# auggiemarignier/pxmcmc

Measured on AMD Instinct MI355X. Metric: MYULA samples/sec at L=256 synthesis, higher is better.
Workload: dtype f64

## Files before the change

include/pxmcmc_amd.h:

```cpp
#ifndef PXMCMC_AMD_H
#define PXMCMC_AMD_H

#include <stddef.h>
#include <stdint.h>

#ifdef __cplusplus
extern "C" {
#endif

typedef struct pxm_sht_plan_s* pxm_sht_plan_t;
typedef struct pxm_wav_plan_s* pxm_wav_plan_t;
typedef struct pxm_dwav_plan_s* pxm_dwav_plan_t;
typedef struct pxm_hwav_plan_s* pxm_hwav_plan_t;
typedef void* pxm_stream_t;

int pxm_version(void);
#ifdef PXM_NOISE_F64
#error "the -DPXM_NOISE_F64 build switch was removed: pass the flag PXM_NOISE_F64 per call (one library serves both precisions)"
#endif
#define PXM_NOISE_F64 16
int pxm_noise_bits(void);
int64_t pxm_host_check_address_ranges(int L, double B, int J_min, int spin, int max_chains, int what);
const char* pxm_last_error(void);
int pxm_device_count(void);

int pxm_capture_begin(void);
int pxm_capture_end(void);
int pxm_deferred_pending(void);
int pxm_tables_trim(void);

int pxm_j_max(int L, double B);
int pxm_wav_bandlimits(int L, double B, int J_min, int* bl_out, int cap);
int64_t pxm_wav_ncoefs(int L, double B, int J_min, int64_t* nscal_out);
int pxm_tiling_axisym(int L, double B, int J_min, double* kappa0, double* kappa);
int pxm_mw_ring_weights(int L, double* q);
int pxm_host_sht_tables(int L, int spin, int m, double* Binv, double* Afwd);
int pxm_host_rec_table(int L, int spin, int m, double* Brec);
// ... 160 lines not shown
```

pxmcmc_amd/_lib.py:

```python
import ctypes as C
import os

import torch

_HERE = os.path.dirname(os.path.abspath(__file__))
LIB_PATH = os.environ.get("PXM_LIB_PATH") or os.path.join(_HERE, "lib", "libpxmcmc_amd.so")

c_i64, c_u64, c_int, c_dbl, c_vp = C.c_int64, C.c_uint64, C.c_int, C.c_double, C.c_void_p

SIGNATURES = {
    "pxm_version": (c_int, []),
    "pxm_noise_bits": (c_int, []),
    "pxm_host_check_address_ranges": (c_i64, [c_int, c_dbl, c_int, c_int, c_int, c_int]),
    "pxm_last_error": (C.c_char_p, []),
    "pxm_device_count": (c_int, []),
    "pxm_capture_begin": (c_int, []),
    "pxm_capture_end": (c_int, []),
    "pxm_deferred_pending": (c_int, []),
    "pxm_tables_trim": (c_int, []),
    "pxm_wav_set_iter_counter": (c_int, [c_vp, c_vp]),
    "pxm_wav_release_iter_counter": (c_int, [c_vp, c_vp]),
    "pxm_wav_iter_counter_add": (c_int, [c_vp, c_u64, c_vp]),
    "pxm_wav_exact_dft_scales": (c_int, [c_vp]),
    "pxm_wav_status": (c_int, [c_vp, c_int, c_vp]),
    "pxm_sht_status": (c_int, [c_vp, c_int, c_vp]),
    "pxm_wav_profile_enable": (c_int, [c_vp, c_int]),
    "pxm_wav_profile_read": (c_int, [c_vp, c_vp, c_vp, c_vp, c_vp]),
    "pxm_wav_profile_read_launches": (c_int, [c_vp, c_vp, c_vp, c_vp, c_i64, c_vp]),
# ... 154 lines not shown
```

pxmcmc_amd/csrc/plans.hip:

```cpp
#include "../../include/pxmcmc_amd.h"
#include "elem.h"
#include "sht_core.h"
#include "sht_rec.h"

#include <algorithm>
#include <cmath>
#include <cstdlib>
#include <cstring>
#include <map>
#include <string>
#include <memory>
#include <mutex>

namespace pxm {

struct TaskList {
  GemmTask* d = nullptr;
  int n = 0;
  bool paired = false;
  int nslab = 2;
  std::vector<int> bls;
  std::vector<int> los;
  double mfma_units = 0;
  bool gram = false;
// ... 82 lines not shown
      if (!any) break;
    }
    v.swap(ordered);
  }
  out->n = (int)v.size();
  out->paired = paired;
  out->nslab = pk ? 4 : (paired ? 2 : 1);
  for (const GemmTask& t : v) {
    PXM_REQUIRE(t.n_rt >= 0 && t.n_rt <= 8 && t.row0 >= 0 && t.row0 % 16 == 0 && t.k_beg >= 0 && t.k_beg % 16 == 0 &&
                    (t.n_rt == 0 || (t.k_end > t.k_beg && (t.k_end - t.k_beg) % 16 == 0)),
                "upload_tasks: malformed GEMM task");
    out->mfma_units += (double)t.n_rt * ((t.k_end - t.k_beg) / 4) * (pk ? 1 : t.nslab);
    for (int sl = 0; sl < 4; ++sl)
      if (t.x2_off[sl]) out->flags |= 1;
    if (t.ks_off[0] || t.ks_off[1]) out->flags |= 2;
  }
  if (v.empty()) return 0;
  if (int rc = check_gemm_task_ranges(v, out->nslab, out->flags, ncol, ws_base, name)) return rc;
  if (int rc = dev_alloc(&out->d, v.size() * sizeof(GemmTask), "GEMM task list")) return rc;
  return dev_upload(out->d, v.data(), v.size() * sizeof(GemmTask));
}

static double tasklist_bytes(const TaskList& tl, int cg) {
  double bytes = 0;
  for (size_t i = 0; i < tl.bls.size(); ++i) {
    const double Ld = tl.bls[i];
    if (tl.gram) bytes += tl.gram_table_bytes + 3 * 16.0 * cg * Ld * Ld + 16.0 * Ld * Ld;
    else bytes += gemm_alg_bytes(tl.bls[i], tl.paired, cg, tl.los[i]);
    if (!tl.gram && tl.pk && tl.tab_shared[i]) bytes -= gemm_table_bytes(tl.bls[i], tl.paired, tl.los[i]);
  }
// ... 238 lines not shown
  double B = 0;
  int nsc = 0;
  std::vector<int> bl;
  std::vector<int64_t> coef_off;
  int64_t ncoefs = 0;
  std::vector<ShtTables*> T;
  ShtTables* TL = nullptr;
  std::vector<DftPlan> dft;
  DftPlan dftL;
  double* ws = nullptr;
  std::vector<int64_t> offG;
  int64_t offGL = 0, offHL = 0, offS = 0;
  int64_t offGD = 0, offHD = 0;
  int64_t offHDc = 0;
  TaskList gram, adj_invadj_D;
  bool have_data_rings = false;
  int64_t offHA = 0, offHB = 0;
  double* d_kc_syn = nullptr;
  double* d_kc_ana = nullptr;
  TaskList syn_fwd, syn_inv, adj_invadj, adj_fwdadj;
  TaskList ana_fwd, ana_inv, anadj_invadj, anadj_fwdadj;
  int64_t table_bytes[2] = {0, 0};
  static constexpr int NSIDE = 3;
  static constexpr int nside = 2;
  hipStream_t side[NSIDE] = {nullptr, nullptr, nullptr};
  hipEvent_t ev_fork = nullptr, ev_join[NSIDE] = {nullptr, nullptr, nullptr};
  bool plain_group = true;
  std::vector<int> lane_of;
  DftGroupList dft_group;
  int pk = 0;
// ... 257 lines not shown

int pxm_wav_plan_create_spin(int L, double B, int J_min, int spin, int max_chains, unsigned flags, pxm_wav_plan_t* plan) {
  (void)flags;
  return wav_plan_create_impl("pxm_wav_plan_create_spin", L, B, J_min, spin, max_chains, plan);
}

int pxm_wav_plan_destroy(pxm_wav_plan_t p) {
  if (!p) return 0;
  dft_group_destroy(&p->dft_group);
  for (auto& d : p->dft) free_dft_plan(&d);
  free_dft_plan(&p->dftL);
  deferred_free(p->ws);
  deferred_free(p->d_kc_syn);
  deferred_free(p->d_kc_ana);
  deferred_free(p->d_wlk);
  deferred_free(p->d_status);
  TaskList* tls[] = {&p->syn_fwd, &p->syn_inv, &p->adj_invadj, &p->adj_fwdadj, &p->gram, &p->adj_invadj_D,
                     &p->ana_fwd, &p->ana_inv, &p->anadj_invadj, &p->anadj_fwdadj, &p->wl_inv, &p->wl_invadj};
  for (TaskList* t : tls) free_tasks(t);
  profiler_release(&p->prof);
  for (ShtTables* T : p->held) release_tables(T);
  rec_tables_destroy(p->rec2);
  deferred_free(p->d_twin);
  deferred_free(p->d_g2n);
  deferred_free(p->d_hn);
  deferred_free(p->d_gn);
  dft_group_destroy(&p->dft_group_n);
  free_tasks(&p->wl_syn_fwd);
  free_tasks(&p->wl_adj_fwdadj);
  delete p;
// ... 353 lines not shown
  if ((rc = launch_ring2px(p->dftL, p->ws + p->offGL, p->ncol, po, C, st))) return rc;
  return pxm_wav_image_init(p, preds_out, data, invcov, invcov_complex, C, stream);
}

}
namespace pxm {
__global__ void k_pack_data_term(const double2* __restrict__ HD, double2* __restrict__ HDc, int64_t rows, int Cp) {
  for (int64_t i = blockIdx.x * (int64_t)blockDim.x + threadIdx.x; i < rows; i += (int64_t)gridDim.x * blockDim.x) HDc[i] = HD[i * Cp];
}
}
extern "C" {

static int wav_make_gram_lists(pxm_wav_plan_t p) {
  int rc;
  if (!p->gram.d) {
    if ((rc = get_tables(p->L, p->spin, 1u << TAB_GRAM, &p->TL))) return rc;
    wav_hold(p, p->TL);
    std::vector<GemmTask> v;
    GemmFuse fz;
    fz.x2_base = p->offHB;
    fz.hd_base = p->offHDc;
    fz.hd_stride = 2;
    append_gemm_tasks(*p->TL, TAB_GRAM, p->ncol, p->offHA, p->L, p->Rp, p->offHL, p->L, p->Rp, nullptr, p->offS, p->ws, v, 0, fz);
    if ((rc = upload_tasks(v, p->TL->paired, &p->gram, {p->L}, p->ncol, p->ws, "Gram step"))) return rc;
    p->gram.gram = true;
    p->gram.gram_table_bytes = (double)p->TL->bytes[TAB_GRAM];
    v.clear();
    append_gemm_tasks(*p->TL, TAB_INV_ADJ, p->ncol, p->offGD, p->L, p->Rp, p->offHD, p->L, p->Rp, nullptr, p->offS, p->ws, v);
    if ((rc = upload_tasks(v, p->TL->paired, &p->adj_invadj_D, {p->L}, p->ncol, p->ws, "inverse-adjoint of the data rings"))) return rc;
  }
  return 0;
}

int pxm_wav_ring_set_data(pxm_wav_plan_t p, const void* data, pxm_stream_t stream) {
  PXM_REQUIRE(p && data, "pxm_wav_ring_set_data: null argument");
  hipStream_t st = (hipStream_t)stream;
  int rc;
  if ((rc = wav_make_gram_lists(p))) return rc;
  PxIn in;
  in.f = (const double*)data;
  in.chain_stride = (int64_t)p->L * (2 * p->L - 1);
// ... 232 lines not shown

int pxm_wav_analysis_adjoint(pxm_wav_plan_t p, const void* X, void* f, int C, pxm_stream_t stream) {
  int rc = wav_check(p, X, f, C, "pxm_wav_analysis_adjoint");
  if (rc) return rc;
  hipStream_t st = (hipStream_t)stream;
  if ((rc = wav_blocks_to_rings(p, X, C, st))) return rc;
  if ((rc = run_tasks(p->anadj_invadj, p->ws, p->ws, p->ncol, C, st, GemmAffine(), &p->prof))) return rc;
  if ((rc = run_tasks(p->anadj_fwdadj, p->ws, p->ws, p->ncol, C, st, GemmAffine(), &p->prof))) return rc;
  PxOut out;
  out.f = (double*)f;
  out.chain_stride = (int64_t)p->L * (2 * p->L - 1);
  return launch_ring2px(p->dftL, p->ws + p->offGL, p->ncol, out, C, st);
}

int64_t pxm_wav_table_bytes(pxm_wav_plan_t p, int op) {
  if (!p || op < 0 || op > 1) return -1;
  return p->table_bytes[op];
}

int64_t pxm_host_check_address_ranges(int L, double B, int J_min, int spin, int max_chains, int what) {
  static std::mutex mu;
  std::lock_guard<std::mutex> lock(mu);
  PXM_REQUIRE(!capture_in_progress(), "pxm_host_check_address_ranges: not during a stream capture");
  set_dry_run(true);
  ranges_checked_reset();
  int rc = 0;
  if (what & 1) {
    pxm_sht_plan_t sp = nullptr;
    rc = pxm_sht_plan_create(L, spin, max_chains, 0, &sp);
    if (sp) pxm_sht_plan_destroy(sp);
  }
  if (!rc && (what & 2)) {
    pxm_wav_plan_t wp = nullptr;
    const int wspin = (what & 8) ? spin : 0;
    rc = pxm_wav_plan_create_spin(L, B, J_min, wspin, max_chains, 0, &wp);
    if (!rc) rc = wav_make_gram_lists(wp);
    if (!rc && (what & 4) && L >= 3 && wspin == 0) rc = pxm_wav_wl_attach(wp, nullptr, nullptr, (int64_t)L * (2 * L - 1));
    if (wp) pxm_wav_plan_destroy(wp);
  }
  tables_trim();
  set_dry_run(false);
  return rc ? -1 : ranges_checked();
}

}
```

pxmcmc_amd/csrc/sht_core.h:

```cpp
#pragma once
#include "common.h"

namespace pxm {

enum TableKind { TAB_INV = 0, TAB_FWD = 1, TAB_INV_ADJ = 2, TAB_FWD_ADJ = 3, TAB_GRAM = 4, TAB_KINDS = 5 };
inline bool kind_el_to_ring(int kind) { return kind == TAB_INV || kind == TAB_FWD_ADJ; }
inline bool kind_rows_are_el(int kind) { return kind == TAB_FWD || kind == TAB_INV_ADJ || kind == TAB_GRAM; }
inline bool kind_k_is_el(int kind) { return kind == TAB_INV || kind == TAB_FWD_ADJ || kind == TAB_GRAM; }

struct GemmTask {
  int64_t tab_off;
  int64_t rt_stride;
  int64_t x_off[4];
  int64_t y_off[4];
  int64_t x2_off[4];
  int64_t hd_off[4];
  int64_t ks_off[2];
  int64_t rs_off[2];
  int row_lo[2], row_hi[2];
  int k_beg, k_end;
  int row0;
  int n_rt;
  int nslab;
  double sign1;
  int m_unit;
  int hd_stride;
  int x_ncol, y_ncol;
};

struct GemmAffine {
  double ns = 0, wr = 0, wi = 0;
  int on = 0;
  int ncol_live = 1 << 30;
  uint64_t* bump = nullptr;
};

struct Profiler {
  struct Pool {
    std::vector<std::pair<hipEvent_t, hipEvent_t>> ev;
    size_t used = 0;
    double bytes = 0, flops = 0;
    std::vector<double> launch_bytes;
// ... 19 lines not shown
                  int32_t* per_launch_wgs = nullptr);
void profiler_release(Profiler* pr);

struct GemmFuse {
  int64_t x2_base = -1;
  const double* rscale = nullptr;
  int row_lo = 0, row_hi = 1 << 30;
  int64_t hd_base = -1;
  int hd_stride = 0;
};

struct ShtTables {
  int L = 0, spin = 0, Rp = 0;
  bool paired = false;
  int n_m = 0;
  double* d_tab[TAB_KINDS] = {nullptr, nullptr, nullptr, nullptr, nullptr};
  size_t bytes[TAB_KINDS] = {0, 0, 0, 0, 0};
  std::vector<int64_t> m_off[TAB_KINDS];
  std::vector<int> k_beg[TAB_KINDS];
  int refs = 0;
  int m_of(int i) const { return paired ? i : i - (L - 1); }
};

int get_tables(int L, int spin, unsigned kinds_mask, ShtTables** out);
void retain_tables(ShtTables* T);
void release_tables(ShtTables* T);
int64_t tables_trim();

void append_gemm_tasks(const ShtTables& T, int kind, int ncol, int64_t x_base, int x_L, int x_Rp,
                       int64_t y_base, int y_L, int y_Rp, const double* kscale, int64_t scratch_off,
                       const double* ws_base, std::vector<GemmTask>& tasks, int el_lo = 0,
                       const GemmFuse& fuse = GemmFuse());
struct GemmSide {
  int64_t x_base, y_base;
  int x_L, x_Rp, y_L, y_Rp;
  const double* kscale;
  int el_lo;
  GemmFuse fuse;
  int x_ncol = 0, y_ncol = 0;
};

void append_gemm_tasks_packed(const ShtTables& T, int kind, int ncol, const GemmSide& side_a, const GemmSide* side_b,
                              int64_t scratch_off, const double* ws_base, std::vector<GemmTask>& tasks);
int launch_gemm_packed(const GemmTask* d_tasks, int n_tasks, int pk, int flags, const double* X, double* Y, int ncol, int col0,
                       double alg_bytes, double flops, hipStream_t stream, Profiler* prof = nullptr);

int launch_gemm(const GemmTask* d_tasks, int n_tasks, int nslab, int flags, const double* X, double* Y, int ncol,
                int col0, int ct, double alg_bytes, double flops, hipStream_t stream,
                const GemmAffine& aff = GemmAffine(), Profiler* prof = nullptr);

inline double gemm_table_bytes(int L, bool paired, int el_lo = 0) {
  double tab_entries = 0;
  for (int m = paired ? 0 : -(L - 1); m < L; ++m) {
    const int am = m < 0 ? -m : m;
    const int n = L - (am > el_lo ? am : el_lo);
// ... 111 lines not shown
```

pxmcmc_amd/csrc/sht_gemm.hip:

```cpp
#include "../../include/pxmcmc_amd.h"
#include "sht_core.h"

#include <type_traits>

#include <hip/hip_ext.h>

#include <cstdlib>
#include <map>
#include <mutex>

namespace pxm {

typedef double d4 __attribute__((ext_vector_type(4)));

constexpr int KC = 16;
#define PXM_GEMM_MFMA(ACC, A, B) ACC = __builtin_amdgcn_mfma_f64_16x16x4f64(A, B, ACC, 0, 0, 0);
#ifdef PXM_GEMM_TRACE
__device__ unsigned long long* g_gemm_trace = nullptr;
extern "C" int pxm_debug_set_gemm_trace(unsigned long long* buf) {
  return hipMemcpyToSymbol(HIP_SYMBOL(g_gemm_trace), &buf, sizeof(buf)) == hipSuccess ? 0 : -1;
}
#endif
__device__ __forceinline__ double stage_add(double a, double b, bool on) { return a + (on ? b : 0.0); }
__device__ __forceinline__ double2 stage_add(double2 a, double2 b, bool on) { return double2{a.x + (on ? b.x : 0.0), a.y + (on ? b.y : 0.0)}; }
// ... 8 lines not shown
template <int CT, int NSLAB, int NW, int RT, int NSET, bool TWO, bool SK, int PK = 0>
__device__ __forceinline__ void sht_gemm_body(const GemmTask* __restrict__ tasks, const int bid,
                                              const double* __restrict__ X, double* __restrict__ Y, int ncol, int col0,
                                              const GemmAffine& aff, double (*xs)[KC][GemmGeom<CT, NSLAB>::PITCH]) {
  constexpr int NCT = CT * NSLAB;
  constexpr bool HOIST = TWO;
  constexpr int COLS = GemmGeom<CT, NSLAB>::COLS;
  constexpr int PITCH = GemmGeom<CT, NSLAB>::PITCH;
  constexpr int NT = 64 * NW;
  constexpr int VW = (KC * COLS / 2 >= NT) ? 2 : 1;
  constexpr int NV = KC * COLS / VW;
  constexpr int IT = (NV + NT - 1) / NT;
  const GemmTask t = tasks[bid];
  const int tid = threadIdx.x, lane = tid & 63;
  if (t.n_rt == 0) return;
  const int xn = PK ? t.x_ncol : ncol, yn = PK ? t.y_ncol : ncol;
#ifdef PXM_GEMM_TRACE
  const unsigned long long trace_t0 = wall_clock64();
  unsigned long long trace_t1 = 0, trace_t2 = 0;
  long long trace_c[5] = {0, 0, 0, 0, 0};
#define PXM_GEMM_CSTAMP(K) if (ch == 8) trace_c[K] = clock64();
#else
#define PXM_GEMM_CSTAMP(K)
#endif
  const int wave = __builtin_amdgcn_readfirstlane(tid >> 6);
  const int kq = lane >> 4, cl = lane & 15;
  const int n_my = min(RT, max(0, t.n_rt - RT * wave));
  const int nch = (t.k_end - t.k_beg) / KC;

  const double* sp[IT];
  const double* sp2[IT];
// ... 12 lines not shown
    sp[i] = X + xo + col0 + cin + (int64_t)(t.k_beg + kr) * xn;
    sp2[i] = sp[i];
    skp[i] = sp[i];
    if (TWO) {
      const int64_t x2o = tasks[bid].x2_off[slab];
      if (x2o) sp2[i] = sp[i] + (x2o - xo);
    }
    if (SK) {
      const int64_t ks = tasks[bid].ks_off[slab >> 1];
      if (ks) skp[i] = X + ks + t.k_beg + kr;
    }
    so[i] = kr * PITCH + col;
  }
  const bool two = TWO && t.x2_off[0] != 0;
  const bool has_sk = SK && t.ks_off[0] != 0;
  typedef typename std::conditional<VW == 2, double2, double>::type stage_t;
  stage_t st[NSET - 1][IT], st2[NSET - 1][IT];
  double ssc[NSET - 1][IT];
#define PXM_STAGE_LOAD(SET, CH)                                                                     \
  {                                                                                                 \
    const int cs = min((CH), nch - 1);                                                              \
    _Pragma("unroll") for (int i = 0; i < IT; ++i) {                                                \
      st[SET][i] = *reinterpret_cast<const stage_t*>(sp[i] + (int64_t)cs * KC * xn);                \
      if (TWO) st2[SET][i] = *reinterpret_cast<const stage_t*>(sp2[i] + (int64_t)cs * KC * xn);   \
      if (SK) ssc[SET][i] = skp[i][cs * KC];                                                        \
    }                                                                                               \
  }
#define PXM_STAGE_STORE(SET, BUF)                                                                   \
  _Pragma("unroll") for (int i = 0; i < IT; ++i) {                                                  \
    stage_t v = st[SET][i];                                                                         \
// ... 73 lines not shown
  }
        PXM_MFMA_CHUNK(NCT)
#undef PXM_MFMA_CHUNK
      }
      PXM_GEMM_CSTAMP(3)
    }
  }
#undef PXM_STAGE_LOAD
#undef PXM_STAGE_STORE
#undef PXM_TAB_LOAD
#ifdef PXM_GEMM_TRACE
  trace_t2 = wall_clock64();
#endif

  constexpr int NGRP = PK ? 2 : 1;
  double hdv[RT][NSLAB][4], rsv[RT][NGRP][4];
#pragma unroll
  for (int r = 0; r < RT; ++r) {
    const int rowb = t.row0 + 16 * (r < n_my ? RT * wave + r : 0) + kq;
#pragma unroll
    for (int sl = 0; sl < NSLAB; ++sl)
#pragma unroll
      for (int q = 0; q < 4; ++q)
        hdv[r][sl][q] = (aff.on && t.hd_off[sl]) ? (X + t.hd_off[sl])[(int64_t)(rowb + 4 * q) * t.hd_stride + (cl & 1)] : 0.0;
#pragma unroll
    for (int g = 0; g < NGRP; ++g)
#pragma unroll
      for (int q = 0; q < 4; ++q) rsv[r][g][q] = t.rs_off[g] ? (X + t.rs_off[g])[rowb + 4 * q] : 1.0;
  }
  if constexpr (PK != 0) {
    const int slab = cl / PK, grp = slab >> 1;
    const bool live = slab < t.nslab;
    const double sgn = (slab & 1) ? t.sign1 : 1.0;
    const int64_t yo = tasks[bid].y_off[live ? slab : 0];
    const int row_lo = grp ? t.row_lo[1] : t.row_lo[0], row_hi = grp ? t.row_hi[1] : t.row_hi[0];
#pragma unroll
    for (int r = 0; r < RT; ++r) {
      if (r >= n_my) continue;
      const int rowb = t.row0 + 16 * (RT * wave + r) + kq;
      double* yb = Y + yo + col0 + (cl % PK) + (int64_t)rowb * yn;
#pragma unroll
      for (int q = 0; q < 4; ++q) {
        const int row = rowb + 4 * q;
        const double rs = grp ? rsv[r][NGRP - 1][q] : rsv[r][0][q];
        if (live && row >= row_lo && row < row_hi) yb[(int64_t)(4 * q) * yn] = sgn * rs * acc[r][0][q];
      }
    }
  } else {
#pragma unroll
  for (int r = 0; r < RT; ++r) {
    if (r >= n_my) continue;
#pragma unroll
    for (int c = 0; c < NCT; ++c) {
      const int slab = c / CT, cin = 16 * (c % CT), grp = slab >> 1;
      const double sgn = (slab & 1) ? t.sign1 : 1.0;
      const int rowb = t.row0 + 16 * (RT * wave + r) + kq;
      double* yb = Y + t.y_off[slab] + col0 + cin + cl + (int64_t)rowb * ncol;
#pragma unroll
      for (int q = 0; q < 4; ++q) {
        const int row = rowb + 4 * q;
        double v = acc[r][c][q];
        if (aff.on) {
          const double u = aff.ns * v - hdv[r][slab][q];
          int lo = __double2loint(u), hi = __double2hiint(u);
          lo = __builtin_amdgcn_mov_dpp(lo, 0xB1, 0xF, 0xF, true);
          hi = __builtin_amdgcn_mov_dpp(hi, 0xB1, 0xF, 0xF, true);
          const double pu = __hiloint2double(hi, lo);
          v = (cl & 1) ? (aff.wr * u + aff.wi * pu) : (aff.wr * u - aff.wi * pu);
          if (col0 + cin + cl >= aff.ncol_live) v = 0.0;
        }
        if (row >= t.row_lo[grp] && row < t.row_hi[grp]) yb[(int64_t)(4 * q) * ncol] = sgn * rsv[r][grp][q] * v;
      }
    }
  }
  }
#ifdef PXM_GEMM_TRACE
  __syncthreads();
  if (tid == 0 && g_gemm_trace) {
    unsigned hw, xcc;
    asm volatile("s_getreg_b32 %0, hwreg(HW_REG_HW_ID)" : "=s"(hw));
    asm volatile("s_getreg_b32 %0, hwreg(HW_REG_XCC_ID)" : "=s"(xcc));
    const unsigned long long slot = atomicAdd(g_gemm_trace, 1ull);
    unsigned long long* r = g_gemm_trace + 8 + 8 * slot;
    r[0] = blockIdx.x; r[1] = gridDim.x; r[2] = trace_t0; r[3] = wall_clock64();
    r[4] = ((unsigned long long)(xcc & 0xf) << 32) | hw; r[5] = (unsigned long long)nch | ((unsigned long long)t.n_rt << 16) | ((unsigned long long)aff.on << 32);
    r[6] = trace_t1; r[7] = trace_t2;
// ... 85 lines not shown
    return -1;
  };
  auto ok = [&](int64_t lo, int64_t hi) {
    ++n;
    return lo <= hi && dev_range_ok(ws_base + lo, ws_base + hi + 1, &why);
  };
  const bool TWO = flags & 1, SK = flags & 2;
  for (size_t ti = 0; ti < v.size(); ++ti) {
    const GemmTask& t = v[ti];
    if (t.n_rt == 0) continue;
    const int nch = (t.k_end - t.k_beg) / KC;
    if (!ok(t.tab_off, t.tab_off + (int64_t)(t.n_rt - 1) * t.rt_stride + (int64_t)(2 * (nch - 1) + 1) * 128 + 127))
      return bad(ti, "ring-table stream", 0);
    for (int col0 = 0; col0 < ncol; col0 += 32) {
      const int CT = (ncol - col0 >= 32) ? 2 : 1;
      for (int slab = 0; slab < nslab; ++slab) {
        const int xn = t.x_ncol ? t.x_ncol : ncol, yn = t.y_ncol ? t.y_ncol : ncol;
        const int wx = std::min(16 * CT, xn), wy = std::min(16 * CT, yn);
        const int64_t lo = col0 + (int64_t)t.k_beg * xn, hi = col0 + wx - 1 + (int64_t)(t.k_end - 1) * xn;
        if (!ok(t.x_off[slab] + lo, t.x_off[slab] + hi)) return bad(ti, "operand staging", col0);
        if (TWO && t.x2_off[slab] && !ok(t.x2_off[slab] + lo, t.x2_off[slab] + hi)) return bad(ti, "second operand staging", col0);
        if (SK && t.ks_off[slab >> 1] && !ok(t.ks_off[slab >> 1] + t.k_beg, t.ks_off[slab >> 1] + t.k_end - 1))
          return bad(ti, "operand scale vector", col0);
        const int64_t r_lo = t.row0, r_hi = t.row0 + 16 * t.n_rt - 1;
        if (t.hd_off[slab] && !ok(t.hd_off[slab] + r_lo * t.hd_stride, t.hd_off[slab] + r_hi * t.hd_stride + 1))
          return bad(ti, "affine data term", col0);
        if (t.rs_off[slab >> 1] && !ok(t.rs_off[slab >> 1] + r_lo, t.rs_off[slab >> 1] + r_hi))
          return bad(ti, "per-row output scale", col0);
        const int64_t s_lo = std::max<int64_t>(r_lo, t.row_lo[slab >> 1]), s_hi = std::min<int64_t>(r_hi, (int64_t)t.row_hi[slab >> 1] - 1);
        if (s_lo <= s_hi && !ok(t.y_off[slab] + col0 + s_lo * yn, t.y_off[slab] + col0 + wy - 1 + s_hi * yn))
// ... 115 lines not shown
    const int n_rt_total = (Rp - row_beg) / 16;
    for (int rt = 0; rt < n_rt_total; rt += rpt) {
      GemmTask g;
      g.m_unit = T.paired ? m : m + T.L - 1;
      g.tab_off = (T.d_tab[kind] + T.m_off[kind][i] + tab_skip + (int64_t)rt * rt_stride) - ws_base;
      g.rt_stride = rt_stride;
      for (int s = 0; s < 2; ++s) fill_side(g, s, T, kind, m, ncol, side, scratch_off, ws_base);
      g.nslab = T.paired ? 2 : 1;
      g.k_beg = k_beg;
      g.k_end = k_end;
      g.row0 = row_beg + 16 * rt;
      g.n_rt = std::min(rpt, n_rt_total - rt);
      g.sign1 = (kind == TAB_GRAM) ? 1.0 : ((m & 1) ? -1.0 : 1.0);
      g.x_ncol = side.x_ncol ? side.x_ncol : ncol;
      g.y_ncol = side.y_ncol ? side.y_ncol : ncol;
      tasks.push_back(g);
    }
  }
}

void append_gemm_tasks_packed(const ShtTables& T, int kind, int ncol, const GemmSide& side_a, const GemmSide* side_b,
                              int64_t scratch_off, const double* ws_base, std::vector<GemmTask>& tasks) {
  GemmSide sa = side_a;
  if (side_b) sa.el_lo = std::min(side_a.el_lo, side_b->el_lo);
  const size_t first = tasks.size();
  append_tasks_impl(T, kind, ncol, sa, scratch_off, ws_base, tasks);
  for (size_t i = first; i < tasks.size(); ++i) {
    GemmTask& g = tasks[i];
    const int m = T.paired ? g.m_unit : g.m_unit - (T.L - 1);
    fill_side(g, 0, T, kind, m, ncol, side_a, scratch_off, ws_base);
    fill_side(g, 1, T, kind, m, ncol, side_b ? *side_b : side_a, scratch_off, ws_base);
    g.nslab = side_b ? 4 : 2;
// ... 22 lines not shown
  const double* Q = Qd + (int64_t)par * Rp * Rp;
  double acc = 0;
  for (int tp = 0; tp < L; ++tp) acc += B[(int64_t)tp * Rp + el] * Q[(int64_t)tp * Rp + t];
  Ad[(int64_t)i * Rp * Rp + (int64_t)el * Rp + t] = scale * acc;
}

__global__ void k_build_gram(const double* __restrict__ Bd, double* __restrict__ Gd, int Rp, int L) {
  const int i = blockIdx.z;
  const int r = blockIdx.x * 16 + threadIdx.x, c = blockIdx.y * 16 + threadIdx.y;
  const double* B = Bd + (int64_t)i * Rp * Rp;
  double acc = 0;
  for (int t = 0; t < L; ++t) acc += B[(int64_t)t * Rp + r] * B[(int64_t)t * Rp + c];
  Gd[(int64_t)i * Rp * Rp + (int64_t)r * Rp + c] = acc;
}

__global__ void k_tile_table(const double* __restrict__ D, double* __restrict__ out, int Rp, int row_beg,
                             int k_beg, int transposed) {
  const int nk2 = (Rp - k_beg) / 8;
  const int rt = blockIdx.y;
  const int kk2 = blockIdx.x;
  const int lane = threadIdx.x >> 1, h = threadIdx.x & 1;
  const int row = row_beg + 16 * rt + (lane & 15);
  const int k = k_beg + 8 * kk2 + 4 * h + (lane >> 4);
  const double v = transposed ? D[(int64_t)k * Rp + row] : D[(int64_t)row * Rp + k];
  out[((int64_t)rt * nk2 + kk2) * 128 + threadIdx.x] = v;
}

static std::mutex g_tab_mutex;
static std::map<std::pair<int, int>, ShtTables*> g_tab_cache;

static int build_kind(ShtTables& T, int kind, const double* d_B, const double* d_A, const double* d_G) {
  const int Rp = T.Rp;
  const bool rows_el = kind_rows_are_el(kind), k_el = kind_k_is_el(kind);
  T.m_off[kind].resize(T.n_m);
  T.k_beg[kind].resize(T.n_m);
  int64_t total = 0;
  for (int i = 0; i < T.n_m; ++i) {
    const int elmin = std::max(std::abs(T.m_of(i)), std::abs(T.spin));
    const int kb = round_down(elmin, 16);
    T.k_beg[kind][i] = kb;
    T.m_off[kind][i] = total;
    total += (int64_t)((rows_el ? Rp - kb : Rp) / 16) * ((k_el ? Rp - kb : Rp) / 8) * 128;
  }
  T.bytes[kind] = (size_t)total * sizeof(double);
  if (int rc = dev_alloc(&T.d_tab[kind], T.bytes[kind], "ring table")) return rc;
  if (dry_run()) return 0;
  for (int i = 0; i < T.n_m; ++i) {
    const int kb = T.k_beg[kind][i];
    const double* src;
    int transposed;
    if (kind == TAB_INV) { src = d_B; transposed = 0; }
// ... 35 lines not shown
  unsigned missing = 0;
  for (int k = 0; k < TAB_KINDS; ++k)
    if ((kinds_mask >> k & 1u) && !T->d_tab[k]) missing |= 1u << k;
  if (missing && dry_run()) {
    for (int k = 0; k < TAB_KINDS; ++k)
      if (missing >> k & 1u) {
        int rc = build_kind(*T, k, nullptr, nullptr, nullptr);
        if (rc) return rc;
      }
  } else if (missing) {
    const int Rp = T->Rp;
    const size_t dense = (size_t)T->n_m * Rp * Rp;
    std::vector<double> hB(dense, 0.0);
    const int m0 = T->paired ? 0 : -(L - 1);
    for (int i = 0; i < T->n_m; ++i) wigner_ring_table(L, spin, m0 + i, hB.data() + (size_t)i * Rp * Rp, Rp);
    double *d_B = nullptr, *d_A = nullptr, *d_Q = nullptr, *d_G = nullptr;
    PXM_HIP(hipMalloc(&d_B, dense * sizeof(double)));
    PXM_HIP(hipMemcpy(d_B, hB.data(), dense * sizeof(double), hipMemcpyHostToDevice));
    hB.clear();
    hB.shrink_to_fit();
    if (missing & ((1u << TAB_FWD) | (1u << TAB_FWD_ADJ))) {
      std::vector<double> hQ((size_t)2 * Rp * Rp, 0.0);
      quadrature_gram(L, +1, hQ.data(), Rp);
      quadrature_gram(L, -1, hQ.data() + (size_t)Rp * Rp, Rp);
      PXM_HIP(hipMalloc(&d_Q, hQ.size() * sizeof(double)));
      PXM_HIP(hipMemcpy(d_Q, hQ.data(), hQ.size() * sizeof(double), hipMemcpyHostToDevice));
      PXM_HIP(hipMalloc(&d_A, dense * sizeof(double)));
      dim3 grid(Rp / 16, Rp / 16, T->n_m), block(16, 16);
      hipLaunchKernelGGL(k_build_fwd, grid, block, 0, 0, d_B, d_Q, d_A, Rp, L, 2.0 * M_PI / (2 * L - 1), m0, spin);
      PXM_HIP(hipGetLastError());
    }
    if (missing & (1u << TAB_GRAM)) {
      PXM_HIP(hipMalloc(&d_G, dense * sizeof(double)));
      dim3 grid(Rp / 16, Rp / 16, T->n_m), block(16, 16);
      hipLaunchKernelGGL(k_build_gram, grid, block, 0, 0, d_B, d_G, Rp, L);
      PXM_HIP(hipGetLastError());
    }
    for (int k = 0; k < TAB_KINDS; ++k)
      if (missing >> k & 1u) {
        int rc = build_kind(*T, k, d_B, d_A, d_G);
        if (rc) return rc;
      }
    PXM_HIP(hipDeviceSynchronize());
    PXM_HIP(hipFree(d_B));
    if (d_A) PXM_HIP(hipFree(d_A));
    if (d_Q) PXM_HIP(hipFree(d_Q));
    if (d_G) PXM_HIP(hipFree(d_G));
  }
  *out = T;
  return 0;
}

void retain_tables(ShtTables* T) {
  std::lock_guard<std::mutex> lock(g_tab_mutex);
  if (T) ++T->refs;
}
void release_tables(ShtTables* T) {
  std::lock_guard<std::mutex> lock(g_tab_mutex);
  if (T && T->refs > 0) --T->refs;
}
int64_t tables_trim() {
  std::lock_guard<std::mutex> lock(g_tab_mutex);
// ... 20 lines not shown
```

Baseline: 115,300.

## Split spin-0 Gram table by degree parity with a rank-one pole correction

For spin 0 and L divisible by 32, the Gram step uses a new table kind that keeps only the even-even and odd-odd degree blocks of each per-m Gram matrix. The GEMM tasks stride over the interleaved rows (row_step 2), and for m=0 a rank-one pole correction is computed in shared memory and added in the epilogue. Large m near Rp stay dense. The goal is to roughly halve Gram table bytes and FLOPs in the MYULA step, at the cost of extra kernel complexity, a shared-memory reduction for m=0, and an environment variable switch.

```diff
diff --git a/include/pxmcmc_amd.h b/include/pxmcmc_amd.h
--- a/include/pxmcmc_amd.h
+++ b/include/pxmcmc_amd.h
@@ -21,6 +21,7 @@
 #define PXM_NOISE_F64 16
 int pxm_noise_bits(void);
 int64_t pxm_host_check_address_ranges(int L, double B, int J_min, int spin, int max_chains, int what);
+int64_t pxm_host_gram_table_bytes(int L, int spin, int* parity);
 const char* pxm_last_error(void);
 int pxm_device_count(void);
 
diff --git a/pxmcmc_amd/_lib.py b/pxmcmc_amd/_lib.py
--- a/pxmcmc_amd/_lib.py
+++ b/pxmcmc_amd/_lib.py
@@ -12,6 +12,7 @@
     "pxm_version": (c_int, []),
     "pxm_noise_bits": (c_int, []),
     "pxm_host_check_address_ranges": (c_i64, [c_int, c_dbl, c_int, c_int, c_int, c_int]),
+    "pxm_host_gram_table_bytes": (c_i64, [c_int, c_int, C.POINTER(c_int)]),
     "pxm_last_error": (C.c_char_p, []),
     "pxm_device_count": (c_int, []),
     "pxm_capture_begin": (c_int, []),
diff --git a/pxmcmc_amd/csrc/plans.hip b/pxmcmc_amd/csrc/plans.hip
--- a/pxmcmc_amd/csrc/plans.hip
+++ b/pxmcmc_amd/csrc/plans.hip
@@ -120,6 +120,8 @@
     for (int sl = 0; sl < 4; ++sl)
       if (t.x2_off[sl]) out->flags |= 1;
     if (t.ks_off[0] || t.ks_off[1]) out->flags |= 2;
+    PXM_REQUIRE(pk || t.n_rt == 0 || ((t.row_step == 1 || t.row_step == 2) && t.x_ncol == ncol * t.row_step && t.y_ncol == ncol * t.row_step),
+                "upload_tasks: a task's row stride differs from row_step * ncol");
   }
   if (v.empty()) return 0;
   if (int rc = check_gemm_task_ranges(v, out->nslab, out->flags, ncol, ws_base, name)) return rc;
@@ -388,6 +390,8 @@
   int64_t offGD = 0, offHD = 0;
   int64_t offHDc = 0;
   TaskList gram, adj_invadj_D;
+  bool gram_parity = false;
+  double* d_pole = nullptr;
   bool have_data_rings = false;
   int64_t offHA = 0, offHB = 0;
   double* d_kc_syn = nullptr;
@@ -675,6 +679,7 @@
   deferred_free(p->d_kc_syn);
   deferred_free(p->d_kc_ana);
   deferred_free(p->d_wlk);
+  deferred_free(p->d_pole);
   deferred_free(p->d_status);
   TaskList* tls[] = {&p->syn_fwd, &p->syn_inv, &p->adj_invadj, &p->adj_fwdadj, &p->gram, &p->adj_invadj_D,
                      &p->ana_fwd, &p->ana_inv, &p->anadj_invadj, &p->anadj_fwdadj, &p->wl_inv, &p->wl_invadj};
@@ -1058,17 +1063,30 @@
 static int wav_make_gram_lists(pxm_wav_plan_t p) {
   int rc;
   if (!p->gram.d) {
-    if ((rc = get_tables(p->L, p->spin, 1u << TAB_GRAM, &p->TL))) return rc;
+    const bool par = gram_parity_wanted(p->L, p->spin);
+    const int kind = par ? TAB_GRAM_PAR : TAB_GRAM;
+    p->gram_parity = par;
+    if ((rc = get_tables(p->L, p->spin, 1u << kind, &p->TL))) return rc;
     wav_hold(p, p->TL);
     std::vector<GemmTask> v;
     GemmFuse fz;
     fz.x2_base = p->offHB;
     fz.hd_base = p->offHDc;
     fz.hd_stride = 2;
-    append_gemm_tasks(*p->TL, TAB_GRAM, p->ncol, p->offHA, p->L, p->Rp, p->offHL, p->L, p->Rp, nullptr, p->offS, p->ws, v, 0, fz);
+    if (par) {
+      const int Rh = p->Rp / 2;
+      std::vector<double> u((size_t)p->Rp, 0.0);
+      for (int l = 0; l < p->L; ++l) u[(size_t)(l & 1) * Rh + l / 2] = ((l & 1) ? -1.0 : 1.0) * std::sqrt((2.0 * l + 1.0) / (8.0 * M_PI));
+      if ((rc = dev_alloc(&p->d_pole, u.size() * sizeof(double), "Gram pole vector [2][Rp / 2]"))) return rc;
+      if ((rc = dev_upload(p->d_pole, u.data(), u.size() * sizeof(double)))) return rc;
+      const GemmSide sd{p->offHA, p->offHL, p->L, p->Rp, p->L, p->Rp, nullptr, 0, fz};
+      append_gram_parity_tasks(*p->TL, p->ncol, sd, p->offS, p->d_pole, p->ws, v);
+    } else {
+      append_gemm_tasks(*p->TL, TAB_GRAM, p->ncol, p->offHA, p->L, p->Rp, p->offHL, p->L, p->Rp, nullptr, p->offS, p->ws, v, 0, fz);
+    }
     if ((rc = upload_tasks(v, p->TL->paired, &p->gram, {p->L}, p->ncol, p->ws, "Gram step"))) return rc;
     p->gram.gram = true;
-    p->gram.gram_table_bytes = (double)p->TL->bytes[TAB_GRAM];
+    p->gram.gram_table_bytes = (double)p->TL->bytes[kind];
     v.clear();
     append_gemm_tasks(*p->TL, TAB_INV_ADJ, p->ncol, p->offGD, p->L, p->Rp, p->offHD, p->L, p->Rp, nullptr, p->offS, p->ws, v);
     if ((rc = upload_tasks(v, p->TL->paired, &p->adj_invadj_D, {p->L}, p->ncol, p->ws, "inverse-adjoint of the data rings"))) return rc;
@@ -1331,7 +1349,9 @@
 }
 
 int64_t pxm_wav_table_bytes(pxm_wav_plan_t p, int op) {
-  if (!p || op < 0 || op > 1) return -1;
+  if (!p || op < 0 || op > 3) return -1;
+  if (op == 2) return (int64_t)p->gram.gram_table_bytes;
+  if (op == 3) return p->gram.d ? (p->gram_parity ? 1 : 0) : -1;
   return p->table_bytes[op];
 }
 
@@ -1360,4 +1380,21 @@
   return rc ? -1 : ranges_checked();
 }
 
-}
+int64_t pxm_host_gram_table_bytes(int L, int spin, int* parity) {
+  static std::mutex mu;
+  std::lock_guard<std::mutex> lock(mu);
+  PXM_REQUIRE(L >= 1 && (std::abs(spin) < L || L == 1), "pxm_host_gram_table_bytes: bad (L, spin)");
+  PXM_REQUIRE(!capture_in_progress(), "pxm_host_gram_table_bytes: not during a stream capture");
+  const bool par = gram_parity_wanted(L, spin);
+  const int kind = par ? TAB_GRAM_PAR : TAB_GRAM;
+  set_dry_run(true);
+  ShtTables* T = nullptr;
+  const int rc = get_tables(L, spin, 1u << kind, &T);
+  const int64_t bytes = rc ? -1 : (int64_t)T->bytes[kind];
+  tables_trim();
+  set_dry_run(false);
+  if (parity) *parity = par ? 1 : 0;
+  return bytes;
+}
+
+}
diff --git a/pxmcmc_amd/csrc/sht_core.h b/pxmcmc_amd/csrc/sht_core.h
--- a/pxmcmc_amd/csrc/sht_core.h
+++ b/pxmcmc_amd/csrc/sht_core.h
@@ -3,10 +3,10 @@
 
 namespace pxm {
 
-enum TableKind { TAB_INV = 0, TAB_FWD = 1, TAB_INV_ADJ = 2, TAB_FWD_ADJ = 3, TAB_GRAM = 4, TAB_KINDS = 5 };
+enum TableKind { TAB_INV = 0, TAB_FWD = 1, TAB_INV_ADJ = 2, TAB_FWD_ADJ = 3, TAB_GRAM = 4, TAB_GRAM_PAR = 5, TAB_KINDS = 6 };
 inline bool kind_el_to_ring(int kind) { return kind == TAB_INV || kind == TAB_FWD_ADJ; }
-inline bool kind_rows_are_el(int kind) { return kind == TAB_FWD || kind == TAB_INV_ADJ || kind == TAB_GRAM; }
-inline bool kind_k_is_el(int kind) { return kind == TAB_INV || kind == TAB_FWD_ADJ || kind == TAB_GRAM; }
+inline bool kind_rows_are_el(int kind) { return kind == TAB_FWD || kind == TAB_INV_ADJ || kind == TAB_GRAM || kind == TAB_GRAM_PAR; }
+inline bool kind_k_is_el(int kind) { return kind == TAB_INV || kind == TAB_FWD_ADJ || kind == TAB_GRAM || kind == TAB_GRAM_PAR; }
 
 struct GemmTask {
   int64_t tab_off;
@@ -26,6 +26,10 @@
   int m_unit;
   int hd_stride;
   int x_ncol, y_ncol;
+  int row_step;
+  int64_t pole_u_off;
+  int64_t pole_uo_off;
+  int64_t pole_dx;
 };
 
 struct GemmAffine {
@@ -75,8 +79,8 @@
   int L = 0, spin = 0, Rp = 0;
   bool paired = false;
   int n_m = 0;
-  double* d_tab[TAB_KINDS] = {nullptr, nullptr, nullptr, nullptr, nullptr};
-  size_t bytes[TAB_KINDS] = {0, 0, 0, 0, 0};
+  double* d_tab[TAB_KINDS] = {};
+  size_t bytes[TAB_KINDS] = {};
   std::vector<int64_t> m_off[TAB_KINDS];
   std::vector<int> k_beg[TAB_KINDS];
   int refs = 0;
@@ -100,6 +104,11 @@
   GemmFuse fuse;
   int x_ncol = 0, y_ncol = 0;
 };
+
+void append_gram_parity_tasks(const ShtTables& T, int ncol, const GemmSide& side, int64_t scratch_off, const double* pole_u,
+                              const double* ws_base, std::vector<GemmTask>& tasks);
+bool gram_parity_wanted(int L, int spin);
+inline bool gram_par_dense_m(int Rp, int m) { return m > 0 && m >= Rp - 32; }
 
 void append_gemm_tasks_packed(const ShtTables& T, int kind, int ncol, const GemmSide& side_a, const GemmSide* side_b,
                               int64_t scratch_off, const double* ws_base, std::vector<GemmTask>& tasks);
diff --git a/pxmcmc_amd/csrc/sht_gemm.hip b/pxmcmc_amd/csrc/sht_gemm.hip
--- a/pxmcmc_amd/csrc/sht_gemm.hip
+++ b/pxmcmc_amd/csrc/sht_gemm.hip
@@ -6,6 +6,7 @@
 #include <hip/hip_ext.h>
 
 #include <cstdlib>
+#include <cstring>
 #include <map>
 #include <mutex>
 
@@ -46,7 +47,7 @@
   const GemmTask t = tasks[bid];
   const int tid = threadIdx.x, lane = tid & 63;
   if (t.n_rt == 0) return;
-  const int xn = PK ? t.x_ncol : ncol, yn = PK ? t.y_ncol : ncol;
+  const int xn = PK ? t.x_ncol : ncol * t.row_step, yn = PK ? t.y_ncol : ncol * t.row_step;
 #ifdef PXM_GEMM_TRACE
   const unsigned long long trace_t0 = wall_clock64();
   unsigned long long trace_t1 = 0, trace_t2 = 0;
@@ -89,6 +90,27 @@
   }
   const bool two = TWO && t.x2_off[0] != 0;
   const bool has_sk = SK && t.ks_off[0] != 0;
+
+  constexpr bool POLE = TWO && PK == 0;
+  constexpr int PCW = 16 * CT;
+  __shared__ double pole_red[POLE ? NT : 1], pole_s[POLE ? PCW : 1];
+  const bool pole = POLE && t.pole_u_off != 0;
+  if (pole) {
+    const int pc = tid % PCW, pg = tid / PCW;
+    const double* xq = X + t.x_off[0] + t.pole_dx + col0 + pc;
+    const double* xq2 = two ? X + t.x2_off[0] + t.pole_dx + col0 + pc : xq;
+    const double* uo = X + t.pole_uo_off;
+    double part = 0.0;
+    for (int k = t.k_beg + pg; k < t.k_end; k += NT / PCW) part += uo[k] * (xq[(int64_t)k * xn] + (two ? xq2[(int64_t)k * xn] : 0.0));
+    pole_red[tid] = part;
+    __syncthreads();
+    if (tid < PCW) {
+      double sum = 0.0;
+      for (int g = 0; g < NT / PCW; ++g) sum += pole_red[g * PCW + tid];
+      pole_s[tid] = sum;
+    }
+    __syncthreads();
+  }
   typedef typename std::conditional<VW == 2, double2, double>::type stage_t;
   stage_t st[NSET - 1][IT], st2[NSET - 1][IT];
   double ssc[NSET - 1][IT];
@@ -192,7 +214,7 @@
 #endif
 
   constexpr int NGRP = PK ? 2 : 1;
-  double hdv[RT][NSLAB][4], rsv[RT][NGRP][4];
+  double hdv[RT][NSLAB][4], rsv[RT][NGRP][4], puv[RT][4];
 #pragma unroll
   for (int r = 0; r < RT; ++r) {
     const int rowb = t.row0 + 16 * (r < n_my ? RT * wave + r : 0) + kq;
@@ -205,6 +227,8 @@
     for (int g = 0; g < NGRP; ++g)
 #pragma unroll
       for (int q = 0; q < 4; ++q) rsv[r][g][q] = t.rs_off[g] ? (X + t.rs_off[g])[rowb + 4 * q] : 1.0;
+#pragma unroll
+    for (int q = 0; q < 4; ++q) puv[r][q] = pole ? (X + t.pole_u_off)[rowb + 4 * q] : 0.0;
   }
   if constexpr (PK != 0) {
     const int slab = cl / PK, grp = slab >> 1;
@@ -233,11 +257,12 @@
       const int slab = c / CT, cin = 16 * (c % CT), grp = slab >> 1;
       const double sgn = (slab & 1) ? t.sign1 : 1.0;
       const int rowb = t.row0 + 16 * (RT * wave + r) + kq;
-      double* yb = Y + t.y_off[slab] + col0 + cin + cl + (int64_t)rowb * ncol;
+      double* yb = Y + t.y_off[slab] + col0 + cin + cl + (int64_t)rowb * yn;
 #pragma unroll
       for (int q = 0; q < 4; ++q) {
         const int row = rowb + 4 * q;
         double v = acc[r][c][q];
+        if (pole) v += puv[r][q] * pole_s[cin + cl];
         if (aff.on) {
           const double u = aff.ns * v - hdv[r][slab][q];
           int lo = __double2loint(u), hi = __double2hiint(u);
@@ -247,7 +272,7 @@
           v = (cl & 1) ? (aff.wr * u + aff.wi * pu) : (aff.wr * u - aff.wi * pu);
           if (col0 + cin + cl >= aff.ncol_live) v = 0.0;
         }
-        if (row >= t.row_lo[grp] && row < t.row_hi[grp]) yb[(int64_t)(4 * q) * ncol] = sgn * rsv[r][grp][q] * v;
+        if (row >= t.row_lo[grp] && row < t.row_hi[grp]) yb[(int64_t)(4 * q) * yn] = sgn * rsv[r][grp][q] * v;
       }
     }
   }
@@ -363,6 +388,14 @@
       return bad(ti, "ring-table stream", 0);
     for (int col0 = 0; col0 < ncol; col0 += 32) {
       const int CT = (ncol - col0 >= 32) ? 2 : 1;
+      if (TWO && t.pole_u_off) {
+        const int xn = t.x_ncol ? t.x_ncol : ncol;
+        const int64_t lo = t.pole_dx + col0 + (int64_t)t.k_beg * xn, hi = t.pole_dx + col0 + 16 * CT - 1 + (int64_t)(t.k_end - 1) * xn;
+        if (!ok(t.x_off[0] + lo, t.x_off[0] + hi)) return bad(ti, "pole-term operand", col0);
+        if (t.x2_off[0] && !ok(t.x2_off[0] + lo, t.x2_off[0] + hi)) return bad(ti, "pole-term second operand", col0);
+        if (!ok(t.pole_uo_off + t.k_beg, t.pole_uo_off + t.k_end - 1)) return bad(ti, "pole vector (contraction side)", col0);
+        if (!ok(t.pole_u_off + t.row0, t.pole_u_off + t.row0 + 16 * t.n_rt - 1)) return bad(ti, "pole vector (row side)", col0);
+      }
       for (int slab = 0; slab < nslab; ++slab) {
         const int xn = t.x_ncol ? t.x_ncol : ncol, yn = t.y_ncol ? t.y_ncol : ncol;
         const int wx = std::min(16 * CT, xn), wy = std::min(16 * CT, yn);
@@ -508,8 +541,77 @@
       g.sign1 = (kind == TAB_GRAM) ? 1.0 : ((m & 1) ? -1.0 : 1.0);
       g.x_ncol = side.x_ncol ? side.x_ncol : ncol;
       g.y_ncol = side.y_ncol ? side.y_ncol : ncol;
+      g.pole_u_off = g.pole_uo_off = g.pole_dx = 0;
+      g.row_step = 1;
       tasks.push_back(g);
     }
+  }
+}
+
+bool gram_parity_wanted(int L, int spin) {
+  const char* e = getenv("PXM_GRAM_PARITY");
+  return spin == 0 && L % 32 == 0 && !(e && atoi(e) == 0);
+}
+
+void append_gram_parity_tasks(const ShtTables& T, int ncol, const GemmSide& side, int64_t scratch_off, const double* pole_u,
+                              const double* ws_base, std::vector<GemmTask>& tasks) {
+  const int Rh = T.Rp / 2;
+  const int rpt = gemm_rows_per_task(ncol);
+  for (int i = 0; i < T.n_m; ++i) {
+    const int m = T.m_of(i);
+    if (gram_par_dense_m(T.Rp, m)) {
+      const int kb16 = T.k_beg[TAB_GRAM_PAR][i];
+      GemmTask g;
+      memset(&g, 0, sizeof(g));
+      g.m_unit = m;
+      g.tab_off = (T.d_tab[TAB_GRAM_PAR] + T.m_off[TAB_GRAM_PAR][i]) - ws_base;
+      g.rt_stride = (int64_t)((T.Rp - kb16) / 8) * 128;
+      for (int s = 0; s < 2; ++s) fill_side(g, s, T, TAB_GRAM_PAR, m, ncol, side, scratch_off, ws_base);
+      g.x_ncol = g.y_ncol = ncol;
+      g.row_step = 1;
+      g.nslab = 2;
+      g.k_beg = kb16;
+      g.k_end = T.Rp;
+      g.row0 = kb16;
+      g.n_rt = (T.Rp - kb16) / 16;
+      g.sign1 = 1.0;
+      tasks.push_back(g);
+      continue;
+    }
+    const int kb = T.k_beg[TAB_GRAM_PAR][i];
+    const int np = Rh - kb;
+    if (np <= 0) continue;
+    const int64_t rt_stride = (int64_t)(np / 8) * 128;
+    for (int par = 0; par < 2; ++par)
+      for (int rt = 0; rt < np / 16; rt += rpt) {
+        GemmTask g;
+        memset(&g, 0, sizeof(g));
+        g.m_unit = m;
+        g.tab_off = (T.d_tab[TAB_GRAM_PAR] + T.m_off[TAB_GRAM_PAR][i] + (int64_t)par * np * np + (int64_t)rt * rt_stride) - ws_base;
+        g.rt_stride = rt_stride;
+        for (int s = 0; s < 2; ++s) fill_side(g, s, T, TAB_GRAM_PAR, m, ncol, side, scratch_off, ws_base);
+        for (int s = 0; s < 4; ++s) {
+          g.x_off[s] += (int64_t)par * ncol;
+          g.y_off[s] += (int64_t)par * ncol;
+          if (g.x2_off[s]) g.x2_off[s] += (int64_t)par * ncol;
+          if (g.hd_off[s]) g.hd_off[s] += (int64_t)par * g.hd_stride;
+        }
+        g.hd_stride *= 2;
+        g.x_ncol = g.y_ncol = 2 * ncol;
+        g.row_step = 2;
+        g.nslab = 2;
+        g.k_beg = kb;
+        g.k_end = Rh;
+        g.row0 = kb + 16 * rt;
+        g.n_rt = std::min(rpt, np / 16 - rt);
+        g.sign1 = 1.0;
+        if (m == 0) {
+          g.pole_u_off = (pole_u + (int64_t)par * Rh) - ws_base;
+          g.pole_uo_off = (pole_u + (int64_t)(1 - par) * Rh) - ws_base;
+          g.pole_dx = (int64_t)(1 - 2 * par) * ncol;
+        }
+        tasks.push_back(g);
+      }
   }
 }
 
@@ -562,6 +664,15 @@
   Gd[(int64_t)i * Rp * Rp + (int64_t)r * Rp + c] = acc;
 }
 
+__global__ void k_build_gram_parity(const double* __restrict__ Bd, double* __restrict__ Gp, int Rp, int L) {
+  const int i = blockIdx.z >> 1, par = blockIdx.z & 1, Rh = Rp / 2;
+  const int a = blockIdx.y * 16 + threadIdx.y, b = blockIdx.x * 16 + threadIdx.x;
+  const double* B = Bd + (int64_t)i * Rp * Rp;
+  double acc = 0;
+  for (int t = 0; t < L; ++t) acc += B[(int64_t)t * Rp + par + 2 * a] * B[(int64_t)t * Rp + par + 2 * b];
+  Gp[((int64_t)(2 * i + par) * Rh + a) * Rh + b] = acc;
+}
+
 __global__ void k_tile_table(const double* __restrict__ D, double* __restrict__ out, int Rp, int row_beg,
                              int k_beg, int transposed) {
   const int nk2 = (Rp - k_beg) / 8;
@@ -574,15 +685,57 @@
   out[((int64_t)rt * nk2 + kk2) * 128 + threadIdx.x] = v;
 }
 
+__global__ void k_tile_from_parity(const double* __restrict__ Gp, double* __restrict__ out, int Rp, int kb) {
+  const int nk2 = (Rp - kb) / 8, Rh = Rp / 2;
+  const int rt = blockIdx.y, kk2 = blockIdx.x;
+  const int lane = threadIdx.x >> 1, h = threadIdx.x & 1;
+  const int row = kb + 16 * rt + (lane & 15);
+  const int k = kb + 8 * kk2 + 4 * h + (lane >> 4);
+  const double v = ((row ^ k) & 1) ? 0.0 : Gp[((int64_t)(row & 1) * Rh + (row >> 1)) * Rh + (k >> 1)];
+  out[((int64_t)rt * nk2 + kk2) * 128 + threadIdx.x] = v;
+}
+
 static std::mutex g_tab_mutex;
 static std::map<std::pair<int, int>, ShtTables*> g_tab_cache;
 
 static int build_kind(ShtTables& T, int kind, const double* d_B, const double* d_A, const double* d_G) {
+  PXM_REQUIRE(kind != TAB_GRAM_PAR || (T.paired && T.Rp % 32 == 0), "parity-split Gram table: spin 0 and Rp a multiple of 32 only");
   const int Rp = T.Rp;
   const bool rows_el = kind_rows_are_el(kind), k_el = kind_k_is_el(kind);
   T.m_off[kind].resize(T.n_m);
   T.k_beg[kind].resize(T.n_m);
   int64_t total = 0;
+  if (kind == TAB_GRAM_PAR) {
+    const int Rh = Rp / 2;
+    for (int i = 0; i < T.n_m; ++i) {
+      const int m = T.m_of(i);
+      const bool dense = gram_par_dense_m(Rp, m);
+      const int kb = dense ? round_down(m, 16) : round_down(m, 32) / 2;
+      T.k_beg[kind][i] = kb;
+      T.m_off[kind][i] = total;
+      total += dense ? (int64_t)(Rp - kb) * (Rp - kb) : 2 * (int64_t)(Rh - kb) * (Rh - kb);
+    }
+    T.bytes[kind] = (size_t)total * sizeof(double);
+    if (int rc = dev_alloc(&T.d_tab[kind], T.bytes[kind], "ring table")) return rc;
+    if (dry_run()) return 0;
+    for (int i = 0; i < T.n_m; ++i) {
+      if (gram_par_dense_m(Rp, T.m_of(i))) {
+        const int kb = T.k_beg[kind][i];
+        dim3 grid((Rp - kb) / 8, (Rp - kb) / 16), block(128);
+        hipLaunchKernelGGL(k_tile_from_parity, grid, block, 0, 0, d_G + (int64_t)2 * i * Rh * Rh, T.d_tab[kind] + T.m_off[kind][i], Rp, kb);
+        continue;
+      }
+      for (int par = 0; par < 2; ++par) {
+        const int kb = T.k_beg[kind][i], np = Rh - kb;
+        dim3 grid(np / 8, np / 16), block(128);
+        if (grid.x == 0 || grid.y == 0) continue;
+        hipLaunchKernelGGL(k_tile_table, grid, block, 0, 0, d_G + (int64_t)(2 * i + par) * Rh * Rh,
+                           T.d_tab[kind] + T.m_off[kind][i] + (int64_t)par * np * np, Rh, kb, kb, 0);
+      }
+    }
+    PXM_HIP(hipGetLastError());
+    return 0;
+  }
   for (int i = 0; i < T.n_m; ++i) {
     const int elmin = std::max(std::abs(T.m_of(i)), std::abs(T.spin));
     const int kb = round_down(elmin, 16);
@@ -648,7 +801,7 @@
     std::vector<double> hB(dense, 0.0);
     const int m0 = T->paired ? 0 : -(L - 1);
     for (int i = 0; i < T->n_m; ++i) wigner_ring_table(L, spin, m0 + i, hB.data() + (size_t)i * Rp * Rp, Rp);
-    double *d_B = nullptr, *d_A = nullptr, *d_Q = nullptr, *d_G = nullptr;
+    double *d_B = nullptr, *d_A = nullptr, *d_Q = nullptr, *d_G = nullptr, *d_GP = nullptr;
     PXM_HIP(hipMalloc(&d_B, dense * sizeof(double)));
     PXM_HIP(hipMemcpy(d_B, hB.data(), dense * sizeof(double), hipMemcpyHostToDevice));
     hB.clear();
@@ -670,9 +823,15 @@
       hipLaunchKernelGGL(k_build_gram, grid, block, 0, 0, d_B, d_G, Rp, L);
       PXM_HIP(hipGetLastError());
     }
+    if (missing & (1u << TAB_GRAM_PAR)) {
+      PXM_HIP(hipMalloc(&d_GP, dense / 2 * sizeof(double)));
+      dim3 grid(Rp / 32, Rp / 32, 2 * T->n_m), block(16, 16);
+      hipLaunchKernelGGL(k_build_gram_parity, grid, block, 0, 0, d_B, d_GP, Rp, L);
+      PXM_HIP(hipGetLastError());
+    }
     for (int k = 0; k < TAB_KINDS; ++k)
       if (missing >> k & 1u) {
-        int rc = build_kind(*T, k, d_B, d_A, d_G);
+        int rc = build_kind(*T, k, d_B, d_A, k == TAB_GRAM_PAR ? d_GP : d_G);
         if (rc) return rc;
       }
     PXM_HIP(hipDeviceSynchronize());
@@ -680,6 +839,7 @@
     if (d_A) PXM_HIP(hipFree(d_A));
     if (d_Q) PXM_HIP(hipFree(d_Q));
     if (d_G) PXM_HIP(hipFree(d_G));
+    if (d_GP) PXM_HIP(hipFree(d_GP));
   }
   *out = T;
   return 0;
```

After: 121,600 (median of 6 runs). 1.05x the previous value.
